# gabefreedman/fastfp

Measured on NVIDIA H100. Metric: Fp evals/sec (freqs x pulsars x draws), higher is better.
Workload: dtype f64

## Files before the change

fastfp_b200/csrc/cabi.cu:

```cuda
#include <algorithm>
#include <cmath>
#include <cstring>

#include "../../include/fastfp_b200.h"
#include "ffp_internal.cuh"

namespace ffp {

std::atomic<int64_t> g_launches{0};
std::atomic<int64_t> g_device_bytes{0};
static thread_local std::string t_err;

void set_error(const std::string& msg) { t_err = msg; }
int cuda_fail(cudaError_t e, const char* what) {
  t_err = std::string("CUDA error: ") + cudaGetErrorString(e) + " in " + what;
  return FASTFP_ERR_CUDA;
}

struct DeviceGuard {
  int prev = -1;
  bool ok = true;
  explicit DeviceGuard(int dev) {
    if (cudaGetDevice(&prev) != cudaSuccess) { prev = -1; }
    if (prev != dev) ok = cudaSetDevice(dev) == cudaSuccess;
// ... 776 lines not shown
    set_error("fastfp_powerlaw_phiinv: invalid argument");
    return FASTFP_ERR_INVALID;
  }
  if (D == 0) return FASTFP_OK;
  PackCall c(pk, stream);
  if (int rc = c.select()) return rc;
  return powerlaw_phiinv_impl(pk, Ffreqs, log10_A, gamma, D, curn_Ffreqs, ncurn, curn_log10_A,
                              curn_gamma, phiinv_var_dev, c.st);
}

static int xcy_run(int device, int64_t n, int64_t m, const double* Nvec, const double* T, const double* sigma,
                   const double* x, const double* y, const double* x0, double* out, void* stream) {
  if (n < 1 || m < 1 || !Nvec || !T || !sigma || !x || !y || !out) {
    set_error("fastfp_xcy: null argument or non-positive size");
    return FASTFP_ERR_INVALID;
  }
  DeviceGuard g(device);
  if (!g.ok) { set_error("cannot select CUDA device " + std::to_string(device)); return FASTFP_ERR_CUDA; }
  cudaStream_t st = (cudaStream_t)stream;
  const size_t tot = (size_t)(4 * n + n * m + m * m) + (size_t)(m * m + 3 * m + 2);
  DeviceBuf<double> d;
  FFP_CUDA(dev_alloc(&d, tot));
  double *dN = d.get(), *dx = dN + n, *dy = dx + n, *dx0 = dy + n, *dT = dx0 + n, *dS = dT + n * m, *dW = dS + m * m;
  double* dO = dW + (m * m + 3 * m);
  cudaError_t e = cudaMemcpyAsync(dN, Nvec, n * 8, cudaMemcpyHostToDevice, st);
  if (e == cudaSuccess) e = cudaMemcpyAsync(dx, x, n * 8, cudaMemcpyHostToDevice, st);
  if (e == cudaSuccess) e = cudaMemcpyAsync(dy, y, n * 8, cudaMemcpyHostToDevice, st);
  if (e == cudaSuccess && x0) e = cudaMemcpyAsync(dx0, x0, n * 8, cudaMemcpyHostToDevice, st);
  if (e == cudaSuccess) e = cudaMemcpyAsync(dT, T, n * m * 8, cudaMemcpyHostToDevice, st);
  if (e == cudaSuccess) e = cudaMemcpyAsync(dS, sigma, m * m * 8, cudaMemcpyHostToDevice, st);
  int rc = 0;
  if (e != cudaSuccess) rc = cuda_fail(e, "fastfp_xcy upload");
  if (!rc) rc = launch_xcy(n, m, dN, dT, dS, dx, dy, x0 ? dx0 : nullptr, dW, dO, st);
  if (!rc) {
    e = cudaMemcpyAsync(out, dO, 8, cudaMemcpyDeviceToHost, st);
    if (e == cudaSuccess) e = cudaStreamSynchronize(st);
    if (e != cudaSuccess) rc = cuda_fail(e, "fastfp_xcy download");
  }
  return rc;
}

int fastfp_xcy(int device, int64_t n, int64_t m, const double* Nvec, const double* T,
               const double* sigma, const double* x, const double* y, double* out, void* stream) {
  return xcy_run(device, n, m, Nvec, T, sigma, x, y, nullptr, out, stream);
}

int fastfp_xcy_blockn(int device, int64_t n, int64_t m, const double* Nvec, const double* T,
                      const double* sigma, const double* x, const double* xw, const double* yw,
                      double* out, void* stream) {
  if (!xw || !yw) { set_error("fastfp_xcy_blockn: null argument"); return FASTFP_ERR_INVALID; }
  return xcy_run(device, n, m, Nvec, T, sigma, xw, yw, x, out, stream);
}

int fastfp_tnt(int device, int64_t n, int64_t m, const double* Nvec, const double* T, const double* phiinv,
               double* out, void* stream) {
  if (n < 1 || m < 1 || !Nvec || !T || !out) {
    set_error("fastfp_tnt: null argument or non-positive size");
    return FASTFP_ERR_INVALID;
  }
  DeviceGuard g(device);
  if (!g.ok) { set_error("cannot select CUDA device " + std::to_string(device)); return FASTFP_ERR_CUDA; }
  cudaStream_t st = (cudaStream_t)stream;
  const int nsplit = (int)std::max<int64_t>(1, std::min<int64_t>(64, n / 256));
  const size_t tot = (size_t)(n + n * m + m + m * m) + (size_t)nsplit * m * m;
  DeviceBuf<double> d;
  FFP_CUDA(dev_alloc(&d, tot));
  double *dN = d.get(), *dT = dN + n, *dP = dT + n * m, *dO = dP + m, *dW = dO + m * m;
  cudaError_t e = cudaMemcpyAsync(dN, Nvec, n * 8, cudaMemcpyHostToDevice, st);
  if (e == cudaSuccess) e = cudaMemcpyAsync(dT, T, n * m * 8, cudaMemcpyHostToDevice, st);
  if (e == cudaSuccess && phiinv) e = cudaMemcpyAsync(dP, phiinv, m * 8, cudaMemcpyHostToDevice, st);
  if (e == cudaSuccess) e = cudaMemsetAsync(dW, 0, (size_t)nsplit * m * m * 8, st);
  int rc = 0;
  if (e != cudaSuccess) rc = cuda_fail(e, "fastfp_tnt upload");
  if (!rc) rc = launch_tnt(n, m, dN, dT, phiinv ? dP : nullptr, dW, nsplit, dO, st);
  if (!rc) {
    e = cudaMemcpyAsync(out, dO, m * m * 8, cudaMemcpyDeviceToHost, st);
    if (e == cudaSuccess) e = cudaStreamSynchronize(st);
    if (e != cudaSuccess) rc = cuda_fail(e, "fastfp_tnt download");
  }
  return rc;
}

int fastfp_fp64_peak(int device, int kind, int iters, double* tflops, double* ms) {
  if (!tflops || !ms || iters < 1 || kind < 0 || kind > 25) {
    set_error("fastfp_fp64_peak: invalid argument");
    return FASTFP_ERR_INVALID;
  }
  DeviceGuard g(device);
  if (!g.ok) { set_error("cannot select CUDA device"); return FASTFP_ERR_CUDA; }
  if (kind == 17 || kind == 18) return run_i8_peak(kind, iters, tflops, ms);
  return run_fp64_peak(kind, iters, tflops, ms);
}

}
```

fastfp_b200/csrc/ffp_internal.cuh:

```cuda
#pragma once
#include <cuda_runtime.h>
#include <stdint.h>

#include <atomic>
#include <map>
#include <memory>
#include <string>
#include <type_traits>
#include <vector>

#include "../../include/fastfp_b200.h"

namespace ffp {

constexpr int NWC = 8;
constexpr int NWP = 16;
constexpr int NTC = NWC * 32, NTP = NWP * 32;
constexpr int CTAS_PER_SM = 1;
constexpr int CONSUMER_REGS = 120, PRODUCER_REGS = 56;
constexpr int VST = 16;
constexpr int FLUSH_TOAS = 512;
constexpr int MAX_M = 640;

inline int sweep_rows(int m, int64_t R, bool blockn) {
  return (m + 7) / 8 * 8 + (int)((R + 7) / 8 * 8) + (blockn ? 8 : 0);
}

template <int NMBW_, int NNB_, int WMW_, int CI_, int NWC_ = ffp::NWC, int NWP_ = ffp::NWP,
          int CREGS_ = CONSUMER_REGS, int PREGS_ = PRODUCER_REGS>
struct SweepCfg {
  static constexpr int NMBW = NMBW_, NNB = NNB_, WMW = WMW_, CI = CI_;
  static constexpr int NWC = NWC_, NWP = NWP_, NTC = NWC_ * 32, NTP = NWP_ * 32, NTHREADS = NTC + NTP;
  static constexpr int CREGS = CREGS_, PREGS = PREGS_;
  static_assert(NTHREADS <= 1024 && NWC % WMW_ == 0, "warp layout");
  static_assert(NTC * CREGS + NTP * PREGS <= NTHREADS * ((65536 / NTHREADS) / 8 * 8), "register pool");
  static constexpr int WNW = NWC / WMW;
  static constexpr int KF = WNW * NNB * 4;
  static constexpr int NMB = NMBW * WMW;
  static constexpr int MP = 8 * NMB;
  static constexpr int KB = CI / 4;
  static constexpr int ST = CI * 2 * KF;
  static constexpr int VEC = 4 * CI;
  static constexpr int GT = CI * MP;
  static constexpr int PK = VEC + GT;
  static constexpr int NX = KF / 8;
  static constexpr int XW = NX >= NWP ? NX / NWP : 1;
  static constexpr int KSPLIT = NX >= ffp::NWP ? 1 : (ffp::NWP / NX < KB ? ffp::NWP / NX : KB);
  static constexpr int KBW = KB / KSPLIT;
  static constexpr int WPG = NX >= NWP ? 1 : (NWP / NX < KSPLIT ? NWP / NX : KSPLIT);
  static constexpr int SPW = KSPLIT / WPG;
  static constexpr int NACTIVE = NX >= NWP ? NWP : NX * WPG;
  static constexpr int NV = PREGS >= 72 ? KBW * XW : 1;
  static constexpr int NACC = 2 * NMBW * NNB;
  static constexpr int NACCX = NACC + 3 * NNB;
  static constexpr int SLAB = NACCX * NTC + 5 * SPW * XW * NTP;
  static constexpr int FLUSH = FLUSH_TOAS / CI;
  static constexpr int SST = ST * 8 * 8 <= 140 * 1024 ? 8 : 4;
  static constexpr int GBUDGET = 214 * 1024 - SST * ST * 8 - VST * VEC * 8;
  static constexpr int GST = GBUDGET / (GT * 8) >= 8 ? 8 : (GBUDGET / (GT * 8) >= 2 ? GBUDGET / (GT * 8) : 2);
  static constexpr int RED = KF * (3 * WMW + 5 * KSPLIT);
  static constexpr size_t SMEM =
      (size_t)(SST * ST + GST * GT + VST * VEC + KF + RED + 2 * (SST + GST + VST)) * 8 + 128;
  static_assert(KB % KSPLIT == 0 && KSPLIT % WPG == 0 && NACTIVE <= NWP && (KBW * XW) % NV == 0,
                "basis-phase mapping");
  static_assert(GST >= 3, "the consumers prefetch across chunk boundaries: three G stages at least");
};

__host__ __device__ inline int g_frag_index(int il, int j, int nmb) {
  return (((il >> 2) * nmb + (j >> 3)) << 5) + (((j & 7) << 2) | (il & 3));
}

struct PulsarMeta {
  int64_t pk_off;
  int64_t L_off;
  int64_t raw_off;
  int64_t T_off;
  int32_t n, m, nch, mpad;
  int32_t mfix, mvar;
  int32_t var_off;
  int32_t ci;
  double tabs_max;
  int64_t dm_off;
  int64_t i8_off;
  int32_t i8_rows;
  int32_t i8_nst;
  double ninv_sum;
};

struct KernelCfg {
  int nmbw, nnb, wmw, ci;
  int nwc = NWC;
  int kf() const { return (nwc / wmw) * nnb * 4; }
  int mp() const { return 8 * nmbw * wmw; }
  bool operator<(const KernelCfg& o) const {
    if (nmbw != o.nmbw) return nmbw < o.nmbw;
    if (nnb != o.nnb) return nnb < o.nnb;
    if (wmw != o.wmw) return wmw < o.wmw;
    if (nwc != o.nwc) return nwc < o.nwc;
    return ci < o.ci;
  }
};

extern std::atomic<int64_t> g_launches;
extern std::atomic<int64_t> g_device_bytes;
void set_error(const std::string& msg);
int cuda_fail(cudaError_t e, const char* what);

#define FFP_CUDA(call)                                         \
  do {                                                         \
    cudaError_t e__ = (call);                                  \
    if (e__ != cudaSuccess) return ffp::cuda_fail(e__, #call); \
  } while (0)

struct CudaFree {
  size_t bytes = 0;
  void operator()(void* p) const {
    cudaFree(p);
    g_device_bytes -= (int64_t)bytes;
  }
};
template <typename T>
using DeviceBuf = std::unique_ptr<T, CudaFree>;
template <typename T>
inline cudaError_t dev_alloc(DeviceBuf<T>* buf, size_t count) {
  T* p = nullptr;
  const size_t bytes = count * sizeof(T);
  const cudaError_t e = cudaMalloc(&p, bytes);
  if (e != cudaSuccess) {
    buf->reset();
    return e;
  }
  g_device_bytes += (int64_t)bytes;
  *buf = DeviceBuf<T>(p, CudaFree{bytes});
  return e;
}
struct CudaFreeHost {
  void operator()(void* p) const { cudaFreeHost(p); }
};
template <typename T>
using PinnedBuf = std::unique_ptr<T, CudaFreeHost>;
template <typename T>
inline cudaError_t pinned_alloc(PinnedBuf<T>* buf, size_t count) {
  T* p = nullptr;
  const cudaError_t e = cudaMallocHost(&p, count * sizeof(T));
  buf->reset(e == cudaSuccess ? p : nullptr);
  return e;
}
struct CudaEventDestroy {
// ... 373 lines not shown
```

fastfp_b200/csrc/fp_sweep_kernel.cuh:

```cuda
#pragma once
#include "ffp_internal.cuh"
#include "ffp_sincos.cuh"

namespace ffp {

enum class SweepMode { Fp, Nmfp, Res };

struct SweepArgs {
  const double* packets;
  const PulsarMeta* meta;
  const int* pidx;
  int ntile_f;
  int nwork;
  const double* freqs;
  int64_t F;
  union {
    FpOut fp;
    NmfpTiles nm;
    ResOut res;
  };
  double* slab;
  unsigned int* counter;
  const unsigned char* done_mask;
#ifdef FFP_DEBUG_SWITCHES
  int dbg;
#endif
};
#ifdef FFP_DEBUG_SWITCHES
#define FFP_DBG(ar, bit) ((ar).dbg & (bit))
#else
#define FFP_DBG(ar, bit) 0
#endif

template <class C>
struct SweepSmem {
  double* Sring;
  double* Gring;
  double* Vring;
  double* fq;
  double* red;
  uint64_t *s_full, *s_empty, *g_full, *g_empty, *v_full, *v_empty;
  __device__ explicit SweepSmem(unsigned char* raw) {
    Sring = reinterpret_cast<double*>(raw);
    Gring = Sring + C::SST * C::ST;
    Vring = Gring + C::GST * C::GT;
    fq = Vring + VST * C::VEC;
    red = fq + C::KF;
    s_full = reinterpret_cast<uint64_t*>(red + C::RED);
    s_empty = s_full + C::SST;
    g_full = s_empty + C::SST;
    g_empty = g_full + C::GST;
    v_full = g_empty + C::GST;
    v_empty = v_full + VST;
  }
};

struct WorkItem {
  int p, ft, nch;
  const double* gpk;
};

template <class C>
__device__ __forceinline__ void producer_loop(const SweepArgs& ar, SweepSmem<C>& sm, volatile int* s_work,
                                              const int pw, const int lane) {
  constexpr int XW = C::XW, SPW = C::SPW, KBW = C::KBW, NV = C::NV;
  const int tidp = pw * 32 + lane;
  const int bk = lane & 3, bf8 = lane >> 2;
  const int bx0 = C::NX >= C::NWP ? pw * XW : pw % C::NX;
  const int bsplit = C::NX >= C::NWP ? 0 : (pw / C::NX) * SPW;
  const int sofs = 2 * lane;
  double* const sl = ar.slab + (size_t)blockIdx.x * C::SLAB + (size_t)C::NACCX * C::NTC + tidp;
  uint32_t g = 0;
  for (;;) {
    __syncthreads();
    const int w = *s_work;
    if (w >= ar.nwork) break;
    const int gp = w / ar.ntile_f;
    const PulsarMeta pm = ar.meta[ar.pidx[gp]];
    const double* gpk = ar.packets + pm.pk_off;
    const int nch = pm.nch;
    auto issue_vec = [&](int c) {
      const uint32_t k = g + (uint32_t)c;
      uint64_t* b = &sm.v_full[k % VST];
      mbar_expect_tx(b, C::VEC * 8);
      tma_load_1d(sm.Vring + (k % VST) * C::VEC, gpk + (size_t)c * C::PK, C::VEC * 8, b);
    };
    if (pw == 0 && lane == 0)
      for (int c = 0; c < VST - 1 && c < nch; ++c) issue_vec(c);
    __syncthreads();
    double omega[XW];
#pragma unroll
    for (int xx = 0; xx < XW; ++xx)
      omega[xx] = __dmul_rn(6.283185307179586, sm.fq[8 * (bx0 + xx) + bf8]);
    bool fast = true;
#pragma unroll
    for (int xx = 0; xx < XW; ++xx) fast = fast && (fabs(omega[xx]) * pm.tabs_max <= 0.999 * FFP_SINCOS_MAX);
    fast = __all_sync(0xffffffffu, fast);
    double s2[SPW][XW][5];
#pragma unroll
    for (int sp = 0; sp < SPW; ++sp)
#pragma unroll
      for (int xx = 0; xx < XW; ++xx)
#pragma unroll
        for (int q = 0; q < 5; ++q) s2[sp][xx][q] = 0.0;
    bool flushed = false;

    for (int c = 0; c < nch; ++c) {
      const uint32_t k = g + (uint32_t)c;
      if (pw == 0 && lane == 0 && c + VST - 2 < nch && c >= 1) {
        if (k >= 2) mbar_wait(&sm.v_empty[(k - 2) % VST], ((k - 2) / VST) & 1u);
        issue_vec(c + VST - 2);
      }
      mbar_wait(&sm.v_full[k % VST], (k / VST) & 1u);
      if (k >= C::SST) mbar_wait(&sm.s_empty[k % C::SST], ((k / C::SST) - 1) & 1u);
      const double* pk = sm.Vring + (k % VST) * C::VEC;
      double* sb = sm.Sring + (k % C::SST) * C::ST + sofs;
      if (!FFP_DBG(ar, 1) && pw < C::NACTIVE) {
#pragma unroll
        for (int sp = 0; sp < SPW; ++sp) {
          const int kb0 = (bsplit + sp) * KBW;
          if (fast) {
#pragma unroll
            for (int e0 = 0; e0 < KBW * XW; e0 += NV) {
              double ph[NV], s[NV], cs[NV], ni[NV], wv[NV];
#pragma unroll
              for (int v = 0; v < NV; ++v) {
                const int i = 4 * (kb0 + (e0 + v) / XW) + bk;
                const double2 tn = *reinterpret_cast<const double2*>(pk + 4 * i);
                ph[v] = __dmul_rn(omega[(e0 + v) % XW], tn.x);
                ni[v] = tn.y;
                wv[v] = pk[4 * i + 2];
              }
              sincos_cw_n<NV>(ph, s, cs);
#pragma unroll
              for (int v = 0; v < NV; ++v) {
                const int kb = kb0 + (e0 + v) / XW, xx = (e0 + v) % XW;
                *reinterpret_cast<double2*>(sb + (kb * C::NX + bx0 + xx) * 64) = make_double2(s[v], cs[v]);
                const double sn = s[v] * ni[v], cn = cs[v] * ni[v];
// ... 251 lines not shown
        }
        flushed = true;
      }
    }
    g += (uint32_t)nch;

    if (flushed) {
      __threadfence();
#pragma unroll
      for (int r = 0; r < NMBW; ++r)
#pragma unroll
        for (int q = 0; q < NMT; ++q)
#pragma unroll
          for (int e = 0; e < 4; ++e)
            if (!(ECORR && r == NMBW - 1 && slot_warp)) acc[r][q][e] += __ldcg(sl + (size_t)((r * NMT + q) * 4 + e) * C::NTC);
      if (ECORR && slot_warp) {
#pragma unroll
        for (int q = 0; q < NMT; ++q)
#pragma unroll
          for (int e = 0; e < 6; ++e) es[q][e / 3][e % 3] += __ldcg(sl + (size_t)(C::NACC + q * 6 + e) * C::NTC);
      }
    }
    const int mfix = pm.mfix;
    double* redB = sm.red;
#pragma unroll
    for (int q = 0; q < NMT; ++q) {
      double ps[2][3] = {{0, 0, 0}, {0, 0, 0}};
#pragma unroll
      for (int r = 0; r < NMBW; ++r)
#pragma unroll
      for (int e = 0; e < 2; ++e) {
        const int j = 8 * (wm * NMBW + r) + 2 * (lane & 3) + e;
        const double ys = acc[r][q][e], yc = acc[r][q][2 + e];
        if (j < mfix) {
          ps[e][0] = fma(ys, ys, ps[e][0]);
          ps[e][1] = fma(ys, yc, ps[e][1]);
          ps[e][2] = fma(yc, yc, ps[e][2]);
        } else if (MODE == SweepMode::Nmfp && j < pm.m) {
          const int64_t f = f0 + 8 * (wn * NMT + q) + (lane >> 2);
          if (f < ar.F) {
            double* z = ar.nm.z(p, f, (ar.F + 31) >> 5, j - mfix + (ar.nm.mvpad - pm.mvar));
            z[0] = ys;
            z[16] = yc;
          }
        }
      }
#pragma unroll
      for (int k = 0; k < 3; ++k) {
        if (ECORR && slot_warp) {
          ps[0][k] += es[q][0][k];
          ps[1][k] += es[q][1][k];
        }
        double v = ps[0][k] + ps[1][k];
        v += __shfl_xor_sync(0xffffffffu, v, 1);
        v += __shfl_xor_sync(0xffffffffu, v, 2);
        if ((lane & 3) == 0) redB[(wm * C::KF + 8 * (wn * NMT + q) + (lane >> 2)) * 3 + k] = v;
      }
    }
    __syncthreads();
    const int64_t fidx = f0 + tid;
    if (tid < C::KF && fidx < ar.F) {
      const double* redA = sm.red + C::WMW * C::KF * 3;
      double b[3] = {0, 0, 0}, a[5] = {0, 0, 0, 0, 0};
      for (int w2 = 0; w2 < C::WMW; ++w2)
#pragma unroll
        for (int k = 0; k < 3; ++k) b[k] += redB[(w2 * C::KF + tid) * 3 + k];
      for (int g2 = 0; g2 < C::KSPLIT; ++g2)
#pragma unroll
        for (int k = 0; k < 5; ++k) a[k] += redA[(g2 * C::KF + tid) * 5 + k];
      if (MODE == SweepMode::Fp) ar.fp.put(p, fidx, ar.F, sm.fq[tid], a[0] - b[0], a[1] - b[1], a[2] - b[2], a[3], a[4]);
      if (MODE == SweepMode::Nmfp) ar.nm.put_a(p, fidx, (ar.F + 31) >> 5, a[0] - b[0], a[1] - b[1], a[2] - b[2], a[3], a[4]);
      if (MODE == SweepMode::Res) {
        redB[tid * 3 + 0] = a[0] - b[0];
        redB[tid * 3 + 1] = a[1] - b[1];
        redB[tid * 3 + 2] = a[2] - b[2];
        ar.res.put_m(p, fidx, sm.fq[tid], a[0] - b[0], a[1] - b[1], a[2] - b[2]);
      }
    }
    if (MODE == SweepMode::Res) res_tail<C>(ar.res, ar.F, sm, acc, redB, p, f0, pm.m, wm, wn, lane);
    __syncthreads();
  }
}

template <class C, SweepMode MODE, bool ECORR>
__global__ void __launch_bounds__(C::NTHREADS, CTAS_PER_SM) fp_sweep_kernel(const SweepArgs ar) {
  extern __shared__ __align__(128) unsigned char smem_raw[];
  SweepSmem<C> sm(smem_raw);
  __shared__ int s_work;
  const int tid = threadIdx.x, lane = tid & 31, wid = tid >> 5;
  if (tid == 0) {
    for (int s = 0; s < C::SST; ++s) { mbar_init(&sm.s_full[s], C::NWP); mbar_init(&sm.s_empty[s], C::NWC); }
    for (int s = 0; s < C::GST; ++s) { mbar_init(&sm.g_full[s], 1); mbar_init(&sm.g_empty[s], C::NWC); }
    for (int s = 0; s < VST; ++s) { mbar_init(&sm.v_full[s], 1); mbar_init(&sm.v_empty[s], C::NWP); }
    fence_barrier_init();
  }
  __syncthreads();
  if (wid < C::NWC) {
    reg_alloc<C::CREGS>();
    consumer_loop<C, MODE, ECORR>(ar, sm, &s_work, wid, lane);
  } else {
    reg_dealloc<C::PREGS>();
    producer_loop<C>(ar, sm, &s_work, wid - C::NWC, lane);
  }
}

template <class C, SweepMode MODE, bool ECORR>
int launch_sweep_cfg(const fastfp_pack* pk, const GroupView& g, const SweepArgs& base, cudaStream_t st) {
  static bool attr_done[64] = {};
  if (!attr_done[pk->device & 63]) {
    FFP_CUDA(cudaFuncSetAttribute(fp_sweep_kernel<C, MODE, ECORR>,
                                  cudaFuncAttributeMaxDynamicSharedMemorySize, (int)C::SMEM));
    attr_done[pk->device & 63] = true;
  }
  SweepArgs a = base;
  a.pidx = g.pidx;
  const int64_t ntile = (a.F + C::KF - 1) / C::KF;
  const int64_t nwork = ntile * g.count;
  if (nwork > 0x7fffffffLL) { set_error("frequency batch too large for one launch"); return -1; }
  a.ntile_f = (int)ntile;
  a.nwork = (int)nwork;
  const int64_t resident = (int64_t)CTAS_PER_SM * pk->num_sms;
  const unsigned grid = (unsigned)(nwork < resident ? nwork : resident);
  FFP_CUDA(cudaMemsetAsync(a.counter, 0, sizeof(unsigned int), st));
  fp_sweep_kernel<C, MODE, ECORR><<<grid, C::NTHREADS, C::SMEM, st>>>(a);
  g_launches += 1;
  FFP_CUDA(cudaGetLastError());
  return 0;
}

int dispatch_sweep_w1(const fastfp_pack*, const GroupView&, const SweepArgs&, SweepMode, cudaStream_t);
int dispatch_sweep_w2(const fastfp_pack*, const GroupView&, const SweepArgs&, SweepMode, cudaStream_t);
int dispatch_sweep_w4(const fastfp_pack*, const GroupView&, const SweepArgs&, SweepMode, cudaStream_t);
int dispatch_sweep_wide(const fastfp_pack*, const GroupView&, const SweepArgs&, SweepMode, cudaStream_t);
int dispatch_sweep_xwide(const fastfp_pack*, const GroupView&, const SweepArgs&, SweepMode, cudaStream_t);

#define FFP_SWEEP_CASE(NMBWv, NNBv, WMWv, CIv) \
  FFP_SWEEP_CASE_W(NMBWv, NNBv, WMWv, CIv, NWC, NWP, CONSUMER_REGS, PRODUCER_REGS)
#define FFP_SWEEP_CASE_W(NMBWv, NNBv, WMWv, CIv, NWCv, NWPv, CREGSv, PREGSv)                       \
  if (g.cfg.nmbw == NMBWv && g.cfg.nnb == NNBv && g.cfg.wmw == WMWv && g.cfg.ci == CIv &&          \
      g.cfg.nwc == NWCv) {                                                                         \
    using Cfg_ = SweepCfg<NMBWv, NNBv, WMWv, CIv, NWCv, NWPv, CREGSv, PREGSv>;                      \
    if (mode == SweepMode::Res)                                                                    \
      return pk->ecorr ? launch_sweep_cfg<Cfg_, SweepMode::Res, true>(pk, g, a, st)                \
                       : launch_sweep_cfg<Cfg_, SweepMode::Res, false>(pk, g, a, st);              \
    if (mode == SweepMode::Nmfp)                                                                   \
      return pk->ecorr ? launch_sweep_cfg<Cfg_, SweepMode::Nmfp, true>(pk, g, a, st)               \
                       : launch_sweep_cfg<Cfg_, SweepMode::Nmfp, false>(pk, g, a, st);             \
    return pk->ecorr ? launch_sweep_cfg<Cfg_, SweepMode::Fp, true>(pk, g, a, st)                   \
                     : launch_sweep_cfg<Cfg_, SweepMode::Fp, false>(pk, g, a, st);                 \
  }

}
```

fastfp_b200/csrc/fp_sweep_w2.cu:

```cuda
#include "fp_sweep_kernel.cuh"
namespace ffp {
#define FFP_SWEEP_CASE_W2(NMBWv) FFP_SWEEP_CASE_W(NMBWv, 2, 1, 32, 8, 8, 168, 88)
int dispatch_sweep_w2(const fastfp_pack* pk, const GroupView& g, const SweepArgs& a, SweepMode mode, cudaStream_t st) {
  FFP_SWEEP_CASE_W2(6) FFP_SWEEP_CASE_W2(7) FFP_SWEEP_CASE_W2(8) FFP_SWEEP_CASE_W2(9) FFP_SWEEP_CASE_W2(10)
  set_error("no sweep kernel for this configuration (w2)");
  return -3;
}
}
```

fastfp_b200/csrc/microbench.cu:

```cuda
#include "ffp_internal.cuh"
#include "ffp_sincos.cuh"

namespace ffp {

__global__ void __launch_bounds__(256) dfma_peak_kernel(int iters, double seed, double* sink) {
  double a[16];
#pragma unroll
  for (int k = 0; k < 16; ++k) a[k] = seed + k + threadIdx.x * 1e-3;
  const double x = 1.0000001, y = 1e-9;
  for (int it = 0; it < iters; ++it) {
#pragma unroll
    for (int k = 0; k < 16; ++k) a[k] = fma(a[k], x, y);
  }
  double s = 0;
#pragma unroll
  for (int k = 0; k < 16; ++k) s += a[k];
  if (s == 12345.678) sink[0] = s;
}

__global__ void __launch_bounds__(256) dmma_peak_kernel(int iters, double seed, double* sink) {
  double c[8][2];
#pragma unroll
  for (int k = 0; k < 8; ++k) c[k][0] = c[k][1] = seed + k;
  const double a = 1.0 + threadIdx.x * 1e-9, b = 1e-3;
// ... 197 lines not shown
      for (int k = 0; k < 8; ++k)
        asm volatile("mma.sync.aligned.m8n8k4.row.col.f64.f64.f64.f64 {%0,%1}, {%2}, {%3}, {%0,%1};"
                     : "+d"(c[k][0]), "+d"(c[k][1])
                     : "d"(a), "d"(b));
    }
#pragma unroll
    for (int k = 0; k < 8; ++k) s += c[k][0] + c[k][1];
  } else {
    const int itf = (int)((long long)iters * 2 * RATIO256 / 256);
    double a[16];
#pragma unroll
    for (int k = 0; k < 16; ++k) a[k] = seed + k + threadIdx.x * 1e-3;
    const double x = 1.0000001, y = 1e-9;
    for (int it = 0; it < itf; ++it) {
#pragma unroll
      for (int k = 0; k < 16; ++k) a[k] = fma(a[k], x, y);
    }
#pragma unroll
    for (int k = 0; k < 16; ++k) s += a[k];
  }
  if (s == 12345.678) sink[0] = s;
}

__global__ void __launch_bounds__(256) imma_peak_kernel(int iters, int seed, double* sink) {
  int c[8][4];
#pragma unroll
  for (int k = 0; k < 8; ++k) c[k][0] = c[k][1] = c[k][2] = c[k][3] = seed + k;
  const unsigned a0 = 0x01020304u + threadIdx.x, a1 = 0x02030405u, a2 = 0x03040506u, a3 = 0x04050607u;
  const unsigned b0 = 0x01010101u, b1 = 0x02020202u;
  for (int it = 0; it < iters; ++it) {
#pragma unroll
    for (int k = 0; k < 8; ++k)
      asm volatile("mma.sync.aligned.m16n8k32.row.col.s32.s8.s8.s32 {%0,%1,%2,%3}, {%4,%5,%6,%7}, {%8,%9}, {%0,%1,%2,%3};"
                   : "+r"(c[k][0]), "+r"(c[k][1]), "+r"(c[k][2]), "+r"(c[k][3])
                   : "r"(a0), "r"(a1), "r"(a2), "r"(a3), "r"(b0), "r"(b1));
  }
  int s = 0;
#pragma unroll
  for (int k = 0; k < 8; ++k) s += c[k][0] + c[k][1] + c[k][2] + c[k][3];
  if (s == 123456789) sink[0] = (double)s;
}

template <int K>
__device__ __forceinline__ void dmma_m16n8(double (&c)[4], const double (&a)[K / 2], const double (&b)[K / 4]) {
  if constexpr (K == 4)
    asm volatile("mma.sync.aligned.m16n8k4.row.col.f64.f64.f64.f64 {%0,%1,%2,%3}, {%4,%5}, {%6}, {%0,%1,%2,%3};"
                 : "+d"(c[0]), "+d"(c[1]), "+d"(c[2]), "+d"(c[3])
                 : "d"(a[0]), "d"(a[1]), "d"(b[0]));
  else if constexpr (K == 8)
    asm volatile("mma.sync.aligned.m16n8k8.row.col.f64.f64.f64.f64 {%0,%1,%2,%3}, {%4,%5,%6,%7}, {%8,%9}, "
                 "{%0,%1,%2,%3};"
                 : "+d"(c[0]), "+d"(c[1]), "+d"(c[2]), "+d"(c[3])
                 : "d"(a[0]), "d"(a[1]), "d"(a[2]), "d"(a[3]), "d"(b[0]), "d"(b[1]));
  else
    asm volatile("mma.sync.aligned.m16n8k16.row.col.f64.f64.f64.f64 {%0,%1,%2,%3}, "
                 "{%4,%5,%6,%7,%8,%9,%10,%11}, {%12,%13,%14,%15}, {%0,%1,%2,%3};"
                 : "+d"(c[0]), "+d"(c[1]), "+d"(c[2]), "+d"(c[3])
                 : "d"(a[0]), "d"(a[1]), "d"(a[2]), "d"(a[3]), "d"(a[4]), "d"(a[5]), "d"(a[6]), "d"(a[7]), "d"(b[0]),
                   "d"(b[1]), "d"(b[2]), "d"(b[3]));
}

template <int K>
__global__ void __launch_bounds__(256, 2) dmma16_peak_kernel(int iters, double seed, double* sink) {
  double c[8][4];
#pragma unroll
  for (int k = 0; k < 8; ++k)
#pragma unroll
    for (int j = 0; j < 4; ++j) c[k][j] = seed + k + j;
  double a[K / 2], b[K / 4];
#pragma unroll
  for (int k = 0; k < K / 2; ++k) a[k] = 1.0 + (threadIdx.x + k) * 1e-9;
#pragma unroll
  for (int k = 0; k < K / 4; ++k) b[k] = 1e-3 * (k + 1);
  for (int it = 0; it < iters; ++it) {
#pragma unroll
    for (int k = 0; k < 8; ++k) dmma_m16n8<K>(c[k], a, b);
  }
  double s = 0;
#pragma unroll
  for (int k = 0; k < 8; ++k) s += c[k][0] + c[k][1] + c[k][2] + c[k][3];
  if (s == 12345.678) sink[0] = s;
}

template <int NWD, int NCH>
__global__ void __launch_bounds__(32 * (8 + NWD), 1) warp_mix16_kernel(int iters, double seed, double* sink) {
  const int w = threadIdx.x >> 5;
  double s = 0;
  if (w < 8) {
    double c[8][4];
#pragma unroll
    for (int k = 0; k < 8; ++k) c[k][0] = c[k][1] = c[k][2] = c[k][3] = seed + k;
    const double a[2] = {1.0 + threadIdx.x * 1e-9, 1.0}, b[1] = {1e-3};
    for (int it = 0; it < iters; ++it) {
#pragma unroll
      for (int k = 0; k < 8; ++k) dmma_m16n8<4>(c[k], a, b);
    }
#pragma unroll
    for (int k = 0; k < 8; ++k) s += c[k][0] + c[k][1] + c[k][2] + c[k][3];
  } else {
    const int itf = (int)((long long)iters * 4 * 50 / 256) * (16 * 16 / (NWD * NCH));
    double a[NCH];
#pragma unroll
    for (int k = 0; k < NCH; ++k) a[k] = seed + k + threadIdx.x * 1e-3;
    const double x = 1.0000001, y = 1e-9;
    for (int it = 0; it < itf; ++it) {
#pragma unroll
      for (int k = 0; k < NCH; ++k) a[k] = fma(a[k], x, y);
    }
#pragma unroll
    for (int k = 0; k < NCH; ++k) s += a[k];
  }
  if (s == 12345.678) sink[0] = s;
}

template <int NMBW, int K>
__global__ void __launch_bounds__(256) dmma16_tile_kernel(int iters, double seed, double* sink) {
  constexpr int KB = K / 4;
  __shared__ double sh[2 * KB * (NMBW + 2) * 32];
  for (int i = threadIdx.x; i < 2 * KB * (NMBW + 2) * 32; i += blockDim.x) sh[i] = seed * 1e-3 + i * 1e-9;
  __syncthreads();
  const int lane = threadIdx.x & 31;
  double acc[NMBW][4];
#pragma unroll
  for (int r = 0; r < NMBW; ++r) acc[r][0] = acc[r][1] = acc[r][2] = acc[r][3] = seed;
  for (int it = 0; it < iters; ++it) {
#pragma unroll
    for (int ks = 0; ks < 2; ++ks) {
      const volatile double* va = sh + ks * KB * (NMBW + 2) * 32;
      double a[K / 2], b[NMBW][K / 4];
#pragma unroll
      for (int kb = 0; kb < KB; ++kb) {
        asm volatile("ld.volatile.shared.v2.f64 {%0, %1}, [%2];"
                     : "=d"(a[2 * kb]), "=d"(a[2 * kb + 1])
                     : "r"(smem_u32((const void*)(va + (kb * (NMBW + 2) + NMBW) * 32 + 2 * lane))));
#pragma unroll
        for (int r = 0; r < NMBW; ++r) b[r][kb] = va[(kb * (NMBW + 2) + r) * 32 + lane];
      }
#pragma unroll
      for (int r = 0; r < NMBW; ++r) dmma_m16n8<K>(acc[r], a, b[r]);
    }
  }
  double s = 0;
#pragma unroll
  for (int r = 0; r < NMBW; ++r) s += acc[r][0] + acc[r][1] + acc[r][2] + acc[r][3];
  if (s == 12345.678) sink[0] = s;
}

int run_fp64_peak(int kind, int iters, double* tflops, double* ms_out) {
  int dev = 0, sms = 0;
  FFP_CUDA(cudaGetDevice(&dev));
  FFP_CUDA(cudaDeviceGetAttribute(&sms, cudaDevAttrMultiProcessorCount, dev));
  DeviceBuf<double> sink_buf;
  FFP_CUDA(dev_alloc(&sink_buf, 1));
  double* sink = sink_buf.get();
  Event ev0, ev1;
  FFP_CUDA(event_create(&ev0));
  FFP_CUDA(event_create(&ev1));
  cudaEvent_t e0 = ev0.get(), e1 = ev1.get();
  const int grid = sms * 8;
  float best = 1e30f;
  if (kind >= 5 && kind <= 8) {
    DeviceBuf<long long> dc_buf;
    FFP_CUDA(dev_alloc(&dc_buf, 1));
    long long* dc = dc_buf.get();
    long long hc = 0;
    for (int rep = 0; rep < 2; ++rep) {
      FFP_CUDA(cudaEventRecord(e0));
      if (kind == 5) dfma_latency_kernel<<<sms, 128>>>(iters, 1.0, sink, dc);
      else if (kind == 6) sincos_rate_kernel<1><<<sms, 256>>>(iters, 1.0, sink, dc);
      else if (kind == 7) sincos_rate_kernel<2><<<sms, 256>>>(iters, 1.0, sink, dc);
      else sincos_rate_kernel<4><<<sms, 256>>>(iters, 1.0, sink, dc);
      FFP_CUDA(cudaEventRecord(e1));
      FFP_CUDA(cudaEventSynchronize(e1));
      FFP_CUDA(cudaEventElapsedTime(&best, e0, e1));
    }
    FFP_CUDA(cudaMemcpy(&hc, dc, 8, cudaMemcpyDeviceToHost));
    g_launches += 2;
    const double per = kind == 5 ? 16.0 * iters : (kind == 6 ? 1.0 : kind == 7 ? 2.0 : 4.0) * iters;
    *tflops = (double)hc / per;
    *ms_out = best;
    return 0;
  }
  for (int rep = 0; rep < 4; ++rep) {
    FFP_CUDA(cudaEventRecord(e0));
    if (kind == 0) dfma_peak_kernel<<<grid, 256>>>(iters, 1.0, sink);
    else if (kind == 19) dmma_peak_kernel<<<grid, 256>>>(iters, 1.0, sink);
    else if (kind == 1) dmma16_peak_kernel<4><<<sms * 2, 256>>>(iters, 1.0, sink);
    else if (kind == 20) dmma16_peak_kernel<8><<<sms * 2, 256>>>(iters, 1.0, sink);
    else if (kind == 21) dmma16_peak_kernel<16><<<sms * 2, 256>>>(iters, 1.0, sink);
    else if (kind == 22) warp_mix16_kernel<16, 16><<<sms, 768>>>(iters, 1.0, sink);
    else if (kind == 25) warp_mix16_kernel<8, 4><<<sms, 512>>>(iters, 1.0, sink);
    else if (kind == 23) dmma16_tile_kernel<9, 4><<<sms, 256>>>(iters, 1.0, sink);
    else if (kind == 24) dmma16_tile_kernel<9, 8><<<sms, 256>>>(iters, 1.0, sink);
    else if (kind == 2) mixed_peak_kernel<<<grid, 256>>>(iters, 1.0, sink);
    else if (kind == 9) dmma_tile_kernel<9, 2><<<sms, 256>>>(iters, 1.0, sink);
    else if (kind == 10) dmma_tile_kernel<9, 2><<<sms, 512>>>(iters, 1.0, sink);
    else if (kind == 11) dmma_tile_kernel<9, 4><<<sms, 128>>>(iters, 1.0, sink);
    else if (kind == 12) dmma_16816_kernel<<<sms, 256>>>(iters, 1.0, sink);
    else if (kind == 16) imma_peak_kernel<<<grid, 256>>>(iters, 1, sink);
    else if (kind == 13) warp_mix_kernel<32><<<sms, 768>>>(iters, 1.0, sink);
    else if (kind == 14) warp_mix_kernel<50><<<sms, 768>>>(iters, 1.0, sink);
    else if (kind == 15) warp_mix_kernel<96><<<sms, 768>>>(iters, 1.0, sink);
    else if (kind == 3) outer_peak_kernel<false><<<sms * 2, 128>>>(iters, 1.0, sink);
    else outer_peak_kernel<true><<<sms * 2, 128>>>(iters, 1.0, sink);
    FFP_CUDA(cudaEventRecord(e1));
    FFP_CUDA(cudaEventSynchronize(e1));
    float ms = 0;
    FFP_CUDA(cudaEventElapsedTime(&ms, e0, e1));
    if (rep > 0 && ms < best) best = ms;
  }
  g_launches += 4;
  FFP_CUDA(cudaGetLastError());
  const double fma_count = kind == 0   ? (double)grid * 256 * 16.0 * iters
                           : kind == 19 ? (double)grid * 8 * 8.0 * 256.0 * iters
                           : kind == 1 || kind == 20 || kind == 21
                               ? (double)sms * 16 * 8 * (128.0 * (kind == 1 ? 4 : kind == 20 ? 8 : 16)) * iters
                           : kind == 22 || kind == 25 ? (double)sms * (8 * 8 * 512.0 * iters +
                                                         16 * 32 * 16.0 * (double)((long long)iters * 4 * 50 / 256))
                           : kind == 23 || kind == 24 ? (double)sms * 8 * 2 * 9 * (128.0 * (kind == 23 ? 4 : 8)) * iters
                           : kind == 9 ? (double)sms * 8 * 2 * 18 * 256.0 * iters
                           : kind == 10 ? (double)sms * 16 * 2 * 18 * 256.0 * iters
                           : kind == 11 ? (double)sms * 4 * 2 * 36 * 256.0 * iters
                           : kind == 12 ? (double)sms * 8 * 4 * 2048.0 * iters
                           : kind == 16 ? (double)grid * 8 * 8.0 * (16.0 * 8 * 32) * iters
                           : kind >= 13 && kind <= 15
                               ? (double)sms * (8 * 8 * 256.0 * iters +
                                                16 * 32 * 16.0 * (double)((long long)iters * 2 * (kind == 13 ? 32 : kind == 14 ? 50 : 96) / 256))
                           : kind == 2 ? (double)grid * (256 * 16.0 + 8 * 4.0 * 256.0) * iters
                                       : (double)sms * 2 * 128 * 144.0 * iters;
  *tflops = 2.0 * fma_count / (best * 1e-3) / 1e12;
  *ms_out = best;
  return 0;
}

}
```

Baseline: 11.56 million.

## Add row-half consumer warp layout for Fp sweep with wider frequency tiles

Adds a row-half (RH=2) consumer mode for the Fp sweep kernel. Pairs of consumer warps split the m-rows of the G tile and each warp covers two m16 frequency tiles (NNB=4), so every loaded G fragment is reused across more MMAs. The two halves combine their partial quadratic forms through a new shared-memory exchange buffer and a named barrier. This raises the per-warp accumulator count and adds cross-warp synchronisation, and it only applies to plain Fp mode with diagonal noise. Microbenchmark kernels are also extended to probe these tile shapes.

```diff
diff --git a/fastfp_b200/csrc/cabi.cu b/fastfp_b200/csrc/cabi.cu
--- a/fastfp_b200/csrc/cabi.cu
+++ b/fastfp_b200/csrc/cabi.cu
@@ -882,7 +882,7 @@
 }
 
 int fastfp_fp64_peak(int device, int kind, int iters, double* tflops, double* ms) {
-  if (!tflops || !ms || iters < 1 || kind < 0 || kind > 25) {
+  if (!tflops || !ms || iters < 1 || kind < 0 || kind > 27) {
     set_error("fastfp_fp64_peak: invalid argument");
     return FASTFP_ERR_INVALID;
   }
diff --git a/fastfp_b200/csrc/ffp_internal.cuh b/fastfp_b200/csrc/ffp_internal.cuh
--- a/fastfp_b200/csrc/ffp_internal.cuh
+++ b/fastfp_b200/csrc/ffp_internal.cuh
@@ -27,14 +27,14 @@
 }
 
 template <int NMBW_, int NNB_, int WMW_, int CI_, int NWC_ = ffp::NWC, int NWP_ = ffp::NWP,
-          int CREGS_ = CONSUMER_REGS, int PREGS_ = PRODUCER_REGS>
+          int CREGS_ = CONSUMER_REGS, int PREGS_ = PRODUCER_REGS, int RH_ = 1>
 struct SweepCfg {
-  static constexpr int NMBW = NMBW_, NNB = NNB_, WMW = WMW_, CI = CI_;
+  static constexpr int NMBW = NMBW_, NNB = NNB_, WMW = WMW_, CI = CI_, RH = RH_;
   static constexpr int NWC = NWC_, NWP = NWP_, NTC = NWC_ * 32, NTP = NWP_ * 32, NTHREADS = NTC + NTP;
   static constexpr int CREGS = CREGS_, PREGS = PREGS_;
-  static_assert(NTHREADS <= 1024 && NWC % WMW_ == 0, "warp layout");
+  static_assert(NTHREADS <= 1024 && NWC % (WMW_ * RH_) == 0 && (RH_ == 1 || (RH_ == 2 && WMW_ == 1)), "warp layout");
   static_assert(NTC * CREGS + NTP * PREGS <= NTHREADS * ((65536 / NTHREADS) / 8 * 8), "register pool");
-  static constexpr int WNW = NWC / WMW;
+  static constexpr int WNW = NWC / (WMW * RH);
   static constexpr int KF = WNW * NNB * 4;
   static constexpr int NMB = NMBW * WMW;
   static constexpr int MP = 8 * NMB;
@@ -51,19 +51,21 @@
   static constexpr int SPW = KSPLIT / WPG;
   static constexpr int NACTIVE = NX >= NWP ? NWP : NX * WPG;
   static constexpr int NV = PREGS >= 72 ? KBW * XW : 1;
-  static constexpr int NACC = 2 * NMBW * NNB;
+  static constexpr int NACC = 2 * ((NMBW + RH - 1) / RH) * NNB;
   static constexpr int NACCX = NACC + 3 * NNB;
   static constexpr int SLAB = NACCX * NTC + 5 * SPW * XW * NTP;
   static constexpr int FLUSH = FLUSH_TOAS / CI;
   static constexpr int SST = ST * 8 * 8 <= 140 * 1024 ? 8 : 4;
-  static constexpr int GBUDGET = 214 * 1024 - SST * ST * 8 - VST * VEC * 8;
+  static constexpr int XF = RH == 1 ? 0 : WNW * 32 * (NNB / 2) * 6;
+  static constexpr int GBUDGET = (RH == 1 ? 214 : 218) * 1024 - SST * ST * 8 - VST * VEC * 8 - XF * 8;
   static constexpr int GST = GBUDGET / (GT * 8) >= 8 ? 8 : (GBUDGET / (GT * 8) >= 2 ? GBUDGET / (GT * 8) : 2);
   static constexpr int RED = KF * (3 * WMW + 5 * KSPLIT);
   static constexpr size_t SMEM =
-      (size_t)(SST * ST + GST * GT + VST * VEC + KF + RED + 2 * (SST + GST + VST)) * 8 + 128;
+      (size_t)(SST * ST + GST * GT + VST * VEC + KF + RED + XF + 2 * (SST + GST + VST)) * 8 + 128;
   static_assert(KB % KSPLIT == 0 && KSPLIT % WPG == 0 && NACTIVE <= NWP && (KBW * XW) % NV == 0,
                 "basis-phase mapping");
   static_assert(GST >= 3, "the consumers prefetch across chunk boundaries: three G stages at least");
+  static_assert(SMEM <= 227 * 1024, "shared memory");
 };
 
 __host__ __device__ inline int g_frag_index(int il, int j, int nmb) {
diff --git a/fastfp_b200/csrc/fp_sweep_kernel.cuh b/fastfp_b200/csrc/fp_sweep_kernel.cuh
--- a/fastfp_b200/csrc/fp_sweep_kernel.cuh
+++ b/fastfp_b200/csrc/fp_sweep_kernel.cuh
@@ -39,6 +39,7 @@
   double* Vring;
   double* fq;
   double* red;
+  double* xf;
   uint64_t *s_full, *s_empty, *g_full, *g_empty, *v_full, *v_empty;
   __device__ explicit SweepSmem(unsigned char* raw) {
     Sring = reinterpret_cast<double*>(raw);
@@ -46,7 +47,8 @@
     Vring = Gring + C::GST * C::GT;
     fq = Vring + VST * C::VEC;
     red = fq + C::KF;
-    s_full = reinterpret_cast<uint64_t*>(red + C::RED);
+    xf = red + C::RED;
+    s_full = reinterpret_cast<uint64_t*>(xf + C::XF);
     s_empty = s_full + C::SST;
     g_full = s_empty + C::SST;
     g_empty = g_full + C::GST;
@@ -54,6 +56,12 @@
     v_empty = v_full + VST;
   }
 };
+
+__device__ __forceinline__ int thread_index() {
+  int t;
+  asm volatile("mov.u32 %0, %%tid.x;" : "=r"(t));
+  return t;
+}
 
 struct WorkItem {
   int p, ft, nch;
@@ -471,6 +479,200 @@
   }
 }
 
+template <class C, int NR, int R0>
+__device__ __forceinline__ void consumer_loop_rh(const SweepArgs& ar, SweepSmem<C>& sm, volatile int* s_work,
+                                                 const int cw, const int lane) {
+  constexpr int NMT = C::NNB / 2;
+  static_assert(C::RH == 2 && C::WMW == 1 && C::NNB % 2 == 0 && 2 * NR * C::NNB <= C::NACC, "row-half layout");
+  const int tid = cw * 32 + lane;
+  const int wn = cw % C::WNW;
+  double* const sl = ar.slab + (size_t)blockIdx.x * C::SLAB + tid;
+  double* const xf = sm.xf + (wn * NMT * 6) * 32 + lane;
+  uint32_t g = 0;
+  for (;;) {
+    if (tid == 0) *s_work = (int)atomicAdd(ar.counter, 1u);
+    __syncthreads();
+    const int w = *s_work;
+    if (w >= ar.nwork) break;
+    const int gp = w / ar.ntile_f, ft = w - gp * ar.ntile_f;
+    const int p = ar.pidx[gp];
+    const PulsarMeta pm = ar.meta[p];
+    const double* gpk = ar.packets + pm.pk_off;
+    const int nch = pm.nch;
+    const int64_t f0 = (int64_t)ft * C::KF;
+    auto issue_G = [&](int c) {
+      const uint32_t k = g + (uint32_t)c;
+      uint64_t* b = &sm.g_full[k % C::GST];
+      mbar_expect_tx(b, C::GT * 8);
+      tma_load_1d(sm.Gring + (k % C::GST) * C::GT, gpk + (size_t)c * C::PK + C::VEC, C::GT * 8, b);
+    };
+    if (tid == 0)
+      for (int c = 0; c < C::GST - 1 && c < nch; ++c) issue_G(c);
+    if (tid < C::KF) sm.fq[tid] = ar.freqs[f0 + tid < ar.F ? f0 + tid : f0];
+    __syncthreads();
+
+    double acc[NR][NMT][4];
+#pragma unroll
+    for (int r = 0; r < NR; ++r)
+#pragma unroll
+      for (int q = 0; q < NMT; ++q) acc[r][q][0] = acc[r][q][1] = acc[r][q][2] = acc[r][q][3] = 0.0;
+    bool flushed = false;
+
+    double2 a0[NMT];
+    double b0[NR];
+    {
+      const uint32_t k = g;
+      mbar_wait_spin(&sm.g_full[k % C::GST], (k / C::GST) & 1u);
+      mbar_wait_spin(&sm.s_full[k % C::SST], (k / C::SST) & 1u);
+      const double* gt = sm.Gring + (k % C::GST) * C::GT + R0 * 32 + lane;
+      const double* sb = sm.Sring + (k % C::SST) * C::ST + (wn * NMT) * 64 + 2 * lane;
+#pragma unroll
+      for (int r = 0; r < NR; ++r) b0[r] = gt[r * 32];
+#pragma unroll
+      for (int q = 0; q < NMT; ++q) a0[q] = *reinterpret_cast<const double2*>(sb + q * 64);
+    }
+    for (int c = 0; c < nch; ++c) {
+      const uint32_t k = g + (uint32_t)c;
+      if (thread_index() == 0 && c + C::GST - 2 < nch && c >= 1) {
+        if (k >= 2) mbar_wait(&sm.g_empty[(k - 2) % C::GST], ((k - 2) / C::GST) & 1u);
+        issue_G(c + C::GST - 2);
+      }
+      const double* gt = sm.Gring + (k % C::GST) * C::GT + R0 * 32 + lane;
+      const double* sb = sm.Sring + (k % C::SST) * C::ST + (wn * NMT) * 64 + 2 * lane;
+#pragma unroll
+      for (int kb = 0; kb < C::KB; ++kb) {
+        double2 a1[NMT];
+        double b1[NR];
+        if (kb + 1 < C::KB) {
+#pragma unroll
+          for (int r = 0; r < NR; ++r) b1[r] = gt[((kb + 1) * C::NMB + r) * 32];
+#pragma unroll
+          for (int q = 0; q < NMT; ++q) a1[q] = *reinterpret_cast<const double2*>(sb + ((kb + 1) * C::NX + q) * 64);
+        } else if (c + 1 < nch) {
+          const uint32_t k1 = k + 1;
+          mbar_wait_spin(&sm.g_full[k1 % C::GST], (k1 / C::GST) & 1u);
+          mbar_wait_spin(&sm.s_full[k1 % C::SST], (k1 / C::SST) & 1u);
+          const double* gt1 = sm.Gring + (k1 % C::GST) * C::GT + R0 * 32 + lane;
+          const double* sb1 = sm.Sring + (k1 % C::SST) * C::ST + (wn * NMT) * 64 + 2 * lane;
+#pragma unroll
+          for (int r = 0; r < NR; ++r) b1[r] = gt1[r * 32];
+#pragma unroll
+          for (int q = 0; q < NMT; ++q) a1[q] = *reinterpret_cast<const double2*>(sb1 + q * 64);
+        } else {
+#pragma unroll
+          for (int r = 0; r < NR; ++r) b1[r] = 0.0;
+#pragma unroll
+          for (int q = 0; q < NMT; ++q) a1[q] = make_double2(0.0, 0.0);
+        }
+        if (!FFP_DBG(ar, 2)) {
+#pragma unroll
+          for (int r = 0; r < NR; ++r)
+#pragma unroll
+            for (int q = 0; q < NMT; ++q) dmma_m16n8k4(acc[r][q], a0[q].x, a0[q].y, b0[r]);
+        }
+#pragma unroll
+        for (int r = 0; r < NR; ++r) b0[r] = b1[r];
+#pragma unroll
+        for (int q = 0; q < NMT; ++q) a0[q] = a1[q];
+      }
+      __syncwarp();
+      if (lane == 0) {
+        mbar_arrive(&sm.g_empty[k % C::GST]);
+        mbar_arrive(&sm.s_empty[k % C::SST]);
+      }
+      if ((c + 1) % C::FLUSH == 0 && c + 1 < nch && !FFP_DBG(ar, 4)) {
+#pragma unroll
+        for (int r = 0; r < NR; ++r)
+#pragma unroll
+          for (int q = 0; q < NMT; ++q)
+#pragma unroll
+            for (int e = 0; e < 4; ++e) {
+              double* a = sl + (size_t)((r * NMT + q) * 4 + e) * C::NTC;
+              if (flushed) atomicAdd(a, acc[r][q][e]);
+              else __stcg(a, acc[r][q][e]);
+              acc[r][q][e] = 0.0;
+            }
+        flushed = true;
+      }
+    }
+    g += (uint32_t)nch;
+
+    if (flushed) {
+      __threadfence();
+#pragma unroll
+      for (int r = 0; r < NR; ++r)
+#pragma unroll
+        for (int q = 0; q < NMT; ++q)
+#pragma unroll
+          for (int e = 0; e < 4; ++e) acc[r][q][e] += __ldcg(sl + (size_t)((r * NMT + q) * 4 + e) * C::NTC);
+    }
+    const int mfix = pm.mfix;
+    double ps[NMT][2][3];
+    if (R0 == 0) {
+#pragma unroll
+      for (int q = 0; q < NMT; ++q)
+#pragma unroll
+        for (int e = 0; e < 2; ++e) ps[q][e][0] = ps[q][e][1] = ps[q][e][2] = 0.0;
+    } else {
+      asm volatile("bar.sync 1, %0;" ::"n"(C::NTC) : "memory");
+#pragma unroll
+      for (int q = 0; q < NMT; ++q)
+#pragma unroll
+        for (int e = 0; e < 2; ++e)
+#pragma unroll
+          for (int k = 0; k < 3; ++k) ps[q][e][k] = xf[(q * 6 + e * 3 + k) * 32];
+    }
+#pragma unroll
+    for (int q = 0; q < NMT; ++q)
+#pragma unroll
+      for (int r = 0; r < NR; ++r)
+#pragma unroll
+        for (int e = 0; e < 2; ++e) {
+          const int j = 8 * (R0 + r) + 2 * (lane & 3) + e;
+          const double ys = acc[r][q][e], yc = acc[r][q][2 + e];
+          if (j < mfix) {
+            ps[q][e][0] = fma(ys, ys, ps[q][e][0]);
+            ps[q][e][1] = fma(ys, yc, ps[q][e][1]);
+            ps[q][e][2] = fma(yc, yc, ps[q][e][2]);
+          }
+        }
+    double* redB = sm.red;
+    if (R0 == 0) {
+#pragma unroll
+      for (int q = 0; q < NMT; ++q)
+#pragma unroll
+        for (int e = 0; e < 2; ++e)
+#pragma unroll
+          for (int k = 0; k < 3; ++k) xf[(q * 6 + e * 3 + k) * 32] = ps[q][e][k];
+      asm volatile("bar.sync 1, %0;" ::"n"(C::NTC) : "memory");
+    } else {
+#pragma unroll
+      for (int q = 0; q < NMT; ++q)
+#pragma unroll
+        for (int k = 0; k < 3; ++k) {
+          double v = ps[q][0][k] + ps[q][1][k];
+          v += __shfl_xor_sync(0xffffffffu, v, 1);
+          v += __shfl_xor_sync(0xffffffffu, v, 2);
+          if ((lane & 3) == 0) redB[(8 * (wn * NMT + q) + (lane >> 2)) * 3 + k] = v;
+        }
+    }
+    __syncthreads();
+    const int tide = thread_index();
+    const int64_t fidx = f0 + tide;
+    if (tide < C::KF && fidx < ar.F) {
+      const double* redA = sm.red + C::KF * 3;
+      double b[3] = {0, 0, 0}, a[5] = {0, 0, 0, 0, 0};
+#pragma unroll
+      for (int k = 0; k < 3; ++k) b[k] += redB[tide * 3 + k];
+      for (int g2 = 0; g2 < C::KSPLIT; ++g2)
+#pragma unroll
+        for (int k = 0; k < 5; ++k) a[k] += redA[(g2 * C::KF + tide) * 5 + k];
+      ar.fp.put(p, fidx, ar.F, sm.fq[tide], a[0] - b[0], a[1] - b[1], a[2] - b[2], a[3], a[4]);
+    }
+    __syncthreads();
+  }
+}
+
 template <class C, SweepMode MODE, bool ECORR>
 __global__ void __launch_bounds__(C::NTHREADS, CTAS_PER_SM) fp_sweep_kernel(const SweepArgs ar) {
   extern __shared__ __align__(128) unsigned char smem_raw[];
@@ -486,7 +688,14 @@
   __syncthreads();
   if (wid < C::NWC) {
     reg_alloc<C::CREGS>();
-    consumer_loop<C, MODE, ECORR>(ar, sm, &s_work, wid, lane);
+    if constexpr (C::RH == 2) {
+      static_assert(MODE == SweepMode::Fp && !ECORR, "row halves: plain Fp with diagonal N");
+      constexpr int NR0 = (C::NMBW + 1) / 2;
+      if (wid < C::WNW) consumer_loop_rh<C, NR0, 0>(ar, sm, &s_work, wid, lane);
+      else consumer_loop_rh<C, C::NMBW - NR0, NR0>(ar, sm, &s_work, wid, lane);
+    } else {
+      consumer_loop<C, MODE, ECORR>(ar, sm, &s_work, wid, lane);
+    }
   } else {
     reg_dealloc<C::PREGS>();
     producer_loop<C>(ar, sm, &s_work, wid - C::NWC, lane);
diff --git a/fastfp_b200/csrc/fp_sweep_w2.cu b/fastfp_b200/csrc/fp_sweep_w2.cu
--- a/fastfp_b200/csrc/fp_sweep_w2.cu
+++ b/fastfp_b200/csrc/fp_sweep_w2.cu
@@ -1,7 +1,13 @@
 #include "fp_sweep_kernel.cuh"
 namespace ffp {
 #define FFP_SWEEP_CASE_W2(NMBWv) FFP_SWEEP_CASE_W(NMBWv, 2, 1, 32, 8, 8, 168, 88)
+#define FFP_SWEEP_FP_RH(NMBWv)                                                                            \
+  if (g.cfg.nmbw == NMBWv && g.cfg.nnb == 2 && g.cfg.wmw == 1 && g.cfg.ci == 32 && g.cfg.nwc == 8)       \
+    return launch_sweep_cfg<SweepCfg<NMBWv, 4, 1, 32, 8, 8, 168, 88, 2>, SweepMode::Fp, false>(pk, g, a, st);
 int dispatch_sweep_w2(const fastfp_pack* pk, const GroupView& g, const SweepArgs& a, SweepMode mode, cudaStream_t st) {
+  if (mode == SweepMode::Fp && !pk->ecorr) {
+    FFP_SWEEP_FP_RH(6) FFP_SWEEP_FP_RH(7) FFP_SWEEP_FP_RH(8) FFP_SWEEP_FP_RH(9) FFP_SWEEP_FP_RH(10)
+  }
   FFP_SWEEP_CASE_W2(6) FFP_SWEEP_CASE_W2(7) FFP_SWEEP_CASE_W2(8) FFP_SWEEP_CASE_W2(9) FFP_SWEEP_CASE_W2(10)
   set_error("no sweep kernel for this configuration (w2)");
   return -3;
diff --git a/fastfp_b200/csrc/microbench.cu b/fastfp_b200/csrc/microbench.cu
--- a/fastfp_b200/csrc/microbench.cu
+++ b/fastfp_b200/csrc/microbench.cu
@@ -303,23 +303,23 @@
   if (s == 12345.678) sink[0] = s;
 }
 
-template <int NWD, int NCH>
-__global__ void __launch_bounds__(32 * (8 + NWD), 1) warp_mix16_kernel(int iters, double seed, double* sink) {
+template <int NWM, int NAC, int NWD, int NCH>
+__global__ void __launch_bounds__(32 * (NWM + NWD), 1) warp_mix16_kernel(int iters, double seed, double* sink) {
   const int w = threadIdx.x >> 5;
   double s = 0;
-  if (w < 8) {
-    double c[8][4];
-#pragma unroll
-    for (int k = 0; k < 8; ++k) c[k][0] = c[k][1] = c[k][2] = c[k][3] = seed + k;
+  if (w < NWM) {
+    double c[NAC][4];
+#pragma unroll
+    for (int k = 0; k < NAC; ++k) c[k][0] = c[k][1] = c[k][2] = c[k][3] = seed + k;
     const double a[2] = {1.0 + threadIdx.x * 1e-9, 1.0}, b[1] = {1e-3};
     for (int it = 0; it < iters; ++it) {
 #pragma unroll
-      for (int k = 0; k < 8; ++k) dmma_m16n8<4>(c[k], a, b);
-    }
-#pragma unroll
-    for (int k = 0; k < 8; ++k) s += c[k][0] + c[k][1] + c[k][2] + c[k][3];
+      for (int k = 0; k < NAC; ++k) dmma_m16n8<4>(c[k], a, b);
+    }
+#pragma unroll
+    for (int k = 0; k < NAC; ++k) s += c[k][0] + c[k][1] + c[k][2] + c[k][3];
   } else {
-    const int itf = (int)((long long)iters * 4 * 50 / 256) * (16 * 16 / (NWD * NCH));
+    const int itf = (int)((long long)iters * 4 * 50 * NWM * NAC / (256 * 64)) * (16 * 16 / (NWD * NCH));
     double a[NCH];
 #pragma unroll
     for (int k = 0; k < NCH; ++k) a[k] = seed + k + threadIdx.x * 1e-3;
@@ -334,36 +334,45 @@
   if (s == 12345.678) sink[0] = s;
 }
 
-template <int NMBW, int K>
+template <int NMBW, int K, int NMT = 1>
 __global__ void __launch_bounds__(256) dmma16_tile_kernel(int iters, double seed, double* sink) {
   constexpr int KB = K / 4;
-  __shared__ double sh[2 * KB * (NMBW + 2) * 32];
-  for (int i = threadIdx.x; i < 2 * KB * (NMBW + 2) * 32; i += blockDim.x) sh[i] = seed * 1e-3 + i * 1e-9;
+  constexpr int KS = NMBW + 2 * NMT;
+  __shared__ double sh[2 * KB * KS * 32];
+  for (int i = threadIdx.x; i < 2 * KB * KS * 32; i += blockDim.x) sh[i] = seed * 1e-3 + i * 1e-9;
   __syncthreads();
   const int lane = threadIdx.x & 31;
-  double acc[NMBW][4];
-#pragma unroll
-  for (int r = 0; r < NMBW; ++r) acc[r][0] = acc[r][1] = acc[r][2] = acc[r][3] = seed;
+  double acc[NMBW][NMT][4];
+#pragma unroll
+  for (int r = 0; r < NMBW; ++r)
+#pragma unroll
+    for (int q = 0; q < NMT; ++q) acc[r][q][0] = acc[r][q][1] = acc[r][q][2] = acc[r][q][3] = seed;
   for (int it = 0; it < iters; ++it) {
 #pragma unroll
     for (int ks = 0; ks < 2; ++ks) {
-      const volatile double* va = sh + ks * KB * (NMBW + 2) * 32;
-      double a[K / 2], b[NMBW][K / 4];
+      const volatile double* va = sh + ks * KB * KS * 32;
+      double a[NMT][K / 2], b[NMBW][K / 4];
 #pragma unroll
       for (int kb = 0; kb < KB; ++kb) {
-        asm volatile("ld.volatile.shared.v2.f64 {%0, %1}, [%2];"
-                     : "=d"(a[2 * kb]), "=d"(a[2 * kb + 1])
-                     : "r"(smem_u32((const void*)(va + (kb * (NMBW + 2) + NMBW) * 32 + 2 * lane))));
-#pragma unroll
-        for (int r = 0; r < NMBW; ++r) b[r][kb] = va[(kb * (NMBW + 2) + r) * 32 + lane];
+#pragma unroll
+        for (int q = 0; q < NMT; ++q)
+          asm volatile("ld.volatile.shared.v2.f64 {%0, %1}, [%2];"
+                       : "=d"(a[q][2 * kb]), "=d"(a[q][2 * kb + 1])
+                       : "r"(smem_u32((const void*)(va + (kb * KS + NMBW + 2 * q) * 32 + 2 * lane))));
+#pragma unroll
+        for (int r = 0; r < NMBW; ++r) b[r][kb] = va[(kb * KS + r) * 32 + lane];
       }
 #pragma unroll
-      for (int r = 0; r < NMBW; ++r) dmma_m16n8<K>(acc[r], a, b[r]);
-    }
-  }
-  double s = 0;
-#pragma unroll
-  for (int r = 0; r < NMBW; ++r) s += acc[r][0] + acc[r][1] + acc[r][2] + acc[r][3];
+      for (int r = 0; r < NMBW; ++r)
+#pragma unroll
+        for (int q = 0; q < NMT; ++q) dmma_m16n8<K>(acc[r][q], a[q], b[r]);
+    }
+  }
+  double s = 0;
+#pragma unroll
+  for (int r = 0; r < NMBW; ++r)
+#pragma unroll
+    for (int q = 0; q < NMT; ++q) s += acc[r][q][0] + acc[r][q][1] + acc[r][q][2] + acc[r][q][3];
   if (s == 12345.678) sink[0] = s;
 }
 
@@ -409,10 +418,12 @@
     else if (kind == 1) dmma16_peak_kernel<4><<<sms * 2, 256>>>(iters, 1.0, sink);
     else if (kind == 20) dmma16_peak_kernel<8><<<sms * 2, 256>>>(iters, 1.0, sink);
     else if (kind == 21) dmma16_peak_kernel<16><<<sms * 2, 256>>>(iters, 1.0, sink);
-    else if (kind == 22) warp_mix16_kernel<16, 16><<<sms, 768>>>(iters, 1.0, sink);
-    else if (kind == 25) warp_mix16_kernel<8, 4><<<sms, 512>>>(iters, 1.0, sink);
+    else if (kind == 22) warp_mix16_kernel<8, 8, 16, 16><<<sms, 768>>>(iters, 1.0, sink);
+    else if (kind == 25) warp_mix16_kernel<8, 8, 8, 4><<<sms, 512>>>(iters, 1.0, sink);
+    else if (kind == 27) warp_mix16_kernel<4, 18, 8, 4><<<sms, 384>>>(iters, 1.0, sink);
     else if (kind == 23) dmma16_tile_kernel<9, 4><<<sms, 256>>>(iters, 1.0, sink);
     else if (kind == 24) dmma16_tile_kernel<9, 8><<<sms, 256>>>(iters, 1.0, sink);
+    else if (kind == 26) dmma16_tile_kernel<9, 4, 2><<<sms, 128>>>(iters, 1.0, sink);
     else if (kind == 2) mixed_peak_kernel<<<grid, 256>>>(iters, 1.0, sink);
     else if (kind == 9) dmma_tile_kernel<9, 2><<<sms, 256>>>(iters, 1.0, sink);
     else if (kind == 10) dmma_tile_kernel<9, 2><<<sms, 512>>>(iters, 1.0, sink);
@@ -438,7 +449,10 @@
                                ? (double)sms * 16 * 8 * (128.0 * (kind == 1 ? 4 : kind == 20 ? 8 : 16)) * iters
                            : kind == 22 || kind == 25 ? (double)sms * (8 * 8 * 512.0 * iters +
                                                          16 * 32 * 16.0 * (double)((long long)iters * 4 * 50 / 256))
+                           : kind == 27 ? (double)sms * (4 * 18 * 512.0 * iters +
+                                                         16 * 32 * 16.0 * (double)((long long)iters * 4 * 50 * 72 / 16384))
                            : kind == 23 || kind == 24 ? (double)sms * 8 * 2 * 9 * (128.0 * (kind == 23 ? 4 : 8)) * iters
+                           : kind == 26 ? (double)sms * 4 * 2 * 9 * 2 * 512.0 * iters
                            : kind == 9 ? (double)sms * 8 * 2 * 18 * 256.0 * iters
                            : kind == 10 ? (double)sms * 16 * 2 * 18 * 256.0 * iters
                            : kind == 11 ? (double)sms * 4 * 2 * 36 * 256.0 * iters
```

Result: faster. 11.70 million, median of 6 (+1.2%).
